# ehsankharazmi/hp-VPINNs

Measured on AMD Instinct MI355X. Metric: variational-loss iterations/sec, higher is better.
Workload: dtype f64; 1 GPU; Poisson-2D hp-VPINN, 16x16 elements, 20x20 GLL quad/elem, 10x10 test fcns/elem, MLP [2,20,20,20,1] tanh, var_form 1, 320 boundary pts, TF1 Adam (BASELINE config 4); points=102400, residuals=25600, params=921, backend=mfma, parallelism=element-sharded dp1, exchange=none, pass_structure=whole-iteration, kernel_variant=k_iter_fused<L=3,SPLIT=false,QT=true,GS=false>

## Files before the change

hp_vpinns_amd/csrc/kernels_fused.hip:

```cpp
#include <cstdio>
#include <cstdlib>
#include <cstring>
#include <type_traits>

#include "hpv_mfma_dev.h"
#include "hpv_fused_dev.h"

#define FZ_WAVES 4
#define FZ_BLOCK (FZ_WAVES * 64)
#define FZ_PRE_PER_THREAD 4
#define FZ_C 3
#define FZ_SHAPE_CONSTS                                                                                              \
    static constexpr int FZ_QX = QX_, FZ_QY = QY_, FZ_NTX = NTX_, FZ_NTY = NTY_, FZ_NQ = QX_ * QY_, FZ_NR = NTX_ * NTY_; \
    static constexpr int FZ_TPE = FZ_NQ / 16;                                                                        \
    static constexpr int FZ_MAXT = FZ_TPE / 4 + 1;       \
    static_assert(FZ_NQ % 16 == 0 && FZ_TPE % 4 <= 1, "element shape not covered by the whole-iteration kernel");
#define FZ_SHAPES(X) X(20, 20, 10, 10) X(16, 16, 8, 8) X(12, 12, 6, 6)

#ifdef HPV_FZ_TIMING
#define FZ_STAMP(I) fz_t[I] = clock64()
#define FZ_SEG(I) do { const long long t_ = clock64(); fz_seg[I] += t_ - fz_last; fz_last = t_; } while (0)
#else
#define FZ_STAMP(I)
#define FZ_SEG(I)
#endif

template <int L, int QX_, int QY_, int NTX_, int NTY_, bool MULTI = false, int C_ = FZ_C, int TRG_ = FZ_C, int NPART_ = 0>
struct FzLds {
    FZ_SHAPE_CONSTS
    static constexpr int LH = L > 1 ? L - 1 : 0;
    static constexpr int WT = 0;
    static constexpr int BH = WT + LH * MF_KS * 64;
    static constexpr int WR = BH + LH * MF_KS * 64;
    static constexpr int WN = WR + LH * MF_KS * 16;
    static constexpr int WRB = WN + LH * MF_KS * 64;
    static constexpr int W1O = WRB + LH * MF_KS * 16;
    static constexpr int CH = W1O + 4 * MF_KS * 64;
    static constexpr int PK = CH + 2 * FZ_NQ;
    static constexpr int XS = PK;
    static constexpr int XLD = FZ_NQ + 16;
    static constexpr int PKS = C_ > FZ_C ? 10 : 6;
    static constexpr int PP = PK + PKS * L * MF_KS * 64;
    static constexpr int PZ = PP + FZ_WAVES * NPART_ * 64;
    static constexpr int TR = PZ + (NPART_ > 0 ? 0 : FZ_WAVES * LH * MF_KS * 32);
    static constexpr int TR_WAVE = TRG_ * 2 * MF_TRB * MF_LD;
    static constexpr int TRSZ = FZ_WAVES * TR_WAVE;
    static constexpr int NTABS = 2 * FZ_NTX * FZ_QX + 2 * FZ_NTY * FZ_QY;
    static constexpr int AX = MULTI ? TR + TRSZ : TR;
    static constexpr int BY = AX + 2 * FZ_NTX * FZ_QX;
    static constexpr int T = MULTI ? TR : BY + 2 * FZ_NTY * FZ_QY;
    static constexpr int UP = T + 2 * FZ_QY * FZ_NTX;
    static constexpr int U = UP + 2 * FZ_NR;
    static constexpr int S = U + FZ_NR;
    static constexpr int RED = S + 2 * FZ_NTY * FZ_QX;
    static_assert(RED + 16 - TR <= FZ_WAVES * TR_WAVE, "projection scratch fits the transpose region");
    static_assert(3 * XLD <= 4 * L * MF_KS * 64, "the staged coordinates fit the parking slots the GS plan leaves free");
    static constexpr int EPI = NPART_ > 0 ? PK : TR;
    static constexpr int total(int P) { return NPART_ > 0 ? TR + TRSZ : TR + (TRSZ > FZ_WAVES * P ? TRSZ : FZ_WAVES * P) + (MULTI ? NTABS : 0); }
};
template <int L, int QX_, int QY_, int NT2>
struct FzPlan {
    static constexpr bool TIGHT = NT2 > 0 && L == 3 && QX_ * QY_ / 16 > 16;
    static constexpr int TRG = TIGHT ? 1 : (NT2 > 0 ? 2 : FZ_C);
    static constexpr int NPART = TIGHT ? 12 : 0;
};

typedef double v2d __attribute__((ext_vector_type(2)));
template <int L, bool SPLIT, bool QT, bool GS, int QX_, int QY_, int NTX_, int NTY_, bool MULTI = false, int NT2 = 0, bool GEN = false>
__global__ void __launch_bounds__(FZ_BLOCK, 1) k_iter_fused(MfmaArgs g) {
    static_assert(!(SPLIT && QT), "the quarter-tile scheme is for whole elements");
    static_assert(!(MULTI && (SPLIT || GS)), "the element loop is for whole elements on the register stash");
    static_assert(!((NT2 > 0 || GEN) && (GS || MULTI)), "the general forms run on the register stash, one workgroup (or a split) per element");
    static_assert(NT2 == 0 || GEN, "a second-tangent channel is always integrated through the general term weights");
    FZ_SHAPE_CONSTS
    static_assert(!(NT2 > 0 && QT && FZ_TPE % FZ_WAVES != 0), "four channels leave the packed quarter tile no slot for the data points: data-quarter plan only");
    constexpr int C = FZ_C + NT2;
    using PLAN = FzPlan<L, QX_, QY_, NT2>;
    constexpr int TRG = PLAN::TRG;
    constexpr int NPART = PLAN::NPART;
    static_assert(C % TRG == 0, "whole transpose passes");
    static_assert(NPART == 0 || !QT, "the tight plan: whole tiles");
    using M = FzLds<L, QX_, QY_, NTX_, NTY_, MULTI, C, TRG, NPART>;
    static_assert(!GEN || (M::AX == M::TR && 4 <= M::TR_WAVE), "the d-epsilon partials live in wave 0's part of the transpose region (it reads them back itself)");
    constexpr int LH = L > 1 ? L - 1 : 1;
    constexpr int NSV = L * MF_KS;
    extern __shared__ __attribute__((aligned(16))) double lds[];
    const int tid = threadIdx.x, lane = tid & 63;
    const int wv = __builtin_amdgcn_readfirstlane(tid >> 6);
    const int q = lane >> 4, pt = lane & 15;
    const int split = SPLIT ? g.proj_split : 1;
    const long el = SPLIT ? (long)(blockIdx.x % (unsigned)g.proj_n_elem) : (long)blockIdx.x;
    long e = SPLIT ? el + g.elem0 : el;
    const int part = SPLIT ? (int)(blockIdx.x / (unsigned)g.proj_n_elem) : 0;
    const double* __restrict__ th = g.theta;
    const ProjArgs& pa = g.pa;
#ifdef HPV_FZ_TIMING
    long long fz_t[8];
    const long long fz_start = clock64(), fz_wall = wall_clock64();
    long long fz_seg[2 + 2 * L], fz_last = clock64();
    int fz_n_own = 0;
#endif

    [[maybe_unused]] constexpr int TNX = FZ_NTX, TNY = FZ_NTY, TQX = FZ_QX, TQY = FZ_QY;
    const int rnx = pa.pd.ntx, rny = pa.pd.nty, rnr = rnx * rny;
    static_assert(FZ_NTX * FZ_QX == FZ_NTY * FZ_QY, "table staging walks both tables with one index");
    double bo = 0.0;
    auto stage_all = [&](auto th) {
        constexpr int N1 = 4 * MF_KS * 64, IT1 = (N1 + FZ_BLOCK - 1) / FZ_BLOCK;
        constexpr int ITW = (MF_KS * 64 + FZ_BLOCK - 1) / FZ_BLOCK;
        double vwt[L > 1 ? L - 1 : 1][ITW], vbh[L > 1 ? L - 1 : 1][ITW], vwn[L > 1 ? L - 1 : 1][ITW];
        double vwr[L > 1 ? L - 1 : 1], vwrb[L > 1 ? L - 1 : 1], v1[IT1];
#pragma unroll
        for (int i_ = 1; i_ < L; ++i_) {
            const int wo = g.woff[i_], bo_ = g.boff[i_];
#pragma unroll
            for (int it = 0; it < ITW; ++it) {
                const int f = it * FZ_BLOCK + tid, fc = f < MF_KS * 64 ? f : 0;
                const int ln = fc & 63, s_ = fc >> 6;
                vwt[i_ - 1][it] = th[wo + (4 * s_ + (ln >> 4)) * MF_H + (ln & 15)];
                vbh[i_ - 1][it] = th[bo_ + 4 * s_ + (ln >> 4)];
                vwn[i_ - 1][it] = th[wo + (ln & 15) * MF_H + 4 * s_ + (ln >> 4)];
            }
            const int fr = tid < MF_KS * 16 ? tid : 0;
            const int a_ = fr & 3, q_ = (fr >> 2) & 3, s_ = fr >> 4;
            vwr[i_ - 1] = th[wo + (4 * s_ + q_) * MF_H + 16 + a_];
            vwrb[i_ - 1] = th[wo + (16 + a_) * MF_H + 4 * s_ + q_];
        }
        const int w0o = g.woff[0], wLo = g.woff[L], b0o = g.boff[0];
#pragma unroll
        for (int it = 0; it < IT1; ++it) {
            const int f = it * FZ_BLOCK + tid, fc = f < N1 ? f : 0;
            const int ln = fc & 63, s_ = (fc >> 6) % MF_KS, c_ = fc / (64 * MF_KS);
            const int j = 4 * s_ + (ln >> 4);
            v1[it] = th[(c_ < 2 ? w0o + c_ * MF_H : (c_ == 2 ? wLo : b0o)) + j];
        }
        constexpr int NTAB = 2 * TNX * TQX, ITT = (NTAB + FZ_BLOCK - 1) / FZ_BLOCK;
        const int dx0 = pa.pd.t[0].dx, dx1 = pa.pd.t[1].dx, dy0 = pa.pd.t[0].dy, dy1 = pa.pd.t[1].dy;
        double vax[ITT], vby[ITT];
#pragma unroll
        for (int it = 0; it < ITT; ++it) {
            const int f = it * FZ_BLOCK + tid, fc = f < NTAB ? f : 0;
            const int tt_ = fc / (TNX * TQX), ti_ = fc % (TNX * TQX);
            const int rr_ = ti_ / TQX, ii_ = ti_ % TQX;
            const bool ton = !GEN || tt_ == 0 || pa.pd.nterms > 1;
            vax[it] = (rr_ < rnx && ton) ? pa.wtx[((long)(tt_ ? dx1 : dx0) * rnx + rr_) * TQX + ii_] : 0.0;
            vby[it] = (rr_ < rny && ton) ? pa.wty[((long)(tt_ ? dy1 : dy0) * rny + rr_) * TQY + ii_] : 0.0;
        }
#pragma unroll
        for (int i_ = 1; i_ < L; ++i_) {
#pragma unroll
            for (int it = 0; it < ITW; ++it) {
                const int f = it * FZ_BLOCK + tid;
                if (f < MF_KS * 64) {
                    lds[M::WT + (i_ - 1) * MF_KS * 64 + f] = vwt[i_ - 1][it];
                    lds[M::BH + (i_ - 1) * MF_KS * 64 + f] = vbh[i_ - 1][it];
                    lds[M::WN + (i_ - 1) * MF_KS * 64 + f] = vwn[i_ - 1][it];
                }
            }
            if (tid < MF_KS * 16) {
                lds[M::WR + (i_ - 1) * MF_KS * 16 + tid] = vwr[i_ - 1];
                lds[M::WRB + (i_ - 1) * MF_KS * 16 + tid] = vwrb[i_ - 1];
            }
        }
#pragma unroll
        for (int it = 0; it < IT1; ++it) {
            const int f = it * FZ_BLOCK + tid;
            if (f < N1) lds[M::W1O + f] = v1[it];
        }
#pragma unroll
        for (int it = 0; it < ITT; ++it) {
            const int f = it * FZ_BLOCK + tid;
            if (f < NTAB) { lds[M::AX + f] = vax[it]; lds[M::BY + f] = vby[it]; }
        }
        bo = th[g.boff[L]];
    };
    [[maybe_unused]] int pre_failed = -1;
    if constexpr (!GS && !MULTI) {
        if (g.pre_g) {
            double* TH = lds + M::PK;
            const AdamArgs& ad = g.pre_ad;
            const double flag = g.pre_g[g.pre_Ptot + 3];
            const int xe = *ad.xerr;
            const bool failed = !(flag == 0.0) || xe;
            pre_failed = failed ? 1 : 0;
            const double b1p = ad.state[0], b2p = ad.state[1];
            double t0[FZ_PRE_PER_THREAD], g0[FZ_PRE_PER_THREAD], m0[FZ_PRE_PER_THREAD], v0[FZ_PRE_PER_THREAD];
#pragma unroll
            for (int k = 0; k < FZ_PRE_PER_THREAD; ++k) {
                const int idx = tid + k * FZ_BLOCK;
                const bool in = idx < g.P;
                t0[k] = in ? ad.theta[idx] : 0.0; g0[k] = in ? g.pre_g[idx] : 0.0; m0[k] = in ? ad.m[idx] : 0.0; v0[k] = in ? ad.v[idx] : 1.0;
            }
#pragma unroll
            for (int k = 0; k < FZ_PRE_PER_THREAD; ++k) {
                const int idx = tid + k * FZ_BLOCK;
                double m1, v1, t1;
                hpv_adam_one(ad.lr, ad.b1, ad.b2, ad.eps, b1p, b2p, g0[k], m0[k], v0[k], t0[k], m1, v1, t1);
                if (idx < g.P) TH[idx] = failed ? t0[k] : t1;
            }
            if (blockIdx.x == 0 && tid == 0) {
                ad.xerr[1] = failed ? 1 : 0;
                if (failed && !xe) __hip_atomic_store(ad.xerr, 1, __ATOMIC_RELAXED, __HIP_MEMORY_SCOPE_AGENT);
            }
            __syncthreads();
            stage_all((const double*)TH);
        } else {
            stage_all(th);
        }
    } else {
        stage_all(th);
    }
    int xsticky = 0;
    unsigned xtag = 0;
    if constexpr (SPLIT) { xsticky = pre_failed >= 0 ? pre_failed : *g.xerr; xtag = *g.xiter + 1u; }
    double pc0 = pa.coef[e], pc1 = (!GEN || pa.pd.nterms > 1) ? pa.coef[pa.coef_stride + e] : 0.0;
    [[maybe_unused]] auto uni = [](double x) -> double {
        return __hiloint2double(__builtin_amdgcn_readfirstlane(__double2hiint(x)), __builtin_amdgcn_readfirstlane(__double2loint(x)));
    };
    [[maybe_unused]] const double geps = (GEN && pa.eps_ptr) ? uni(pa.eps_ptr[0]) : 0.0;
    [[maybe_unused]] const bool gtwo = GEN && pa.pd.nterms > 1;
    [[maybe_unused]] double WA0[C], WA1[C], WB1[C];
    if constexpr (GEN) {
#pragma unroll
        for (int c = 1; c < C; ++c) {
            const double t1 = uni(fma(geps, pa.pd.t[1].a1[c], pa.pd.t[1].a0[c]));
            WA0[c] = uni(fma(geps, pa.pd.t[0].a1[c], pa.pd.t[0].a0[c]));
            WA1[c] = uni(gtwo ? t1 : pa.pd.t[0].a1[c]);
            WB1[c] = uni(gtwo ? t1 : 0.0);
        }
    }
    [[maybe_unused]] auto wa0 = [&](int c) -> double { return WA0[c]; };
    [[maybe_unused]] auto wa1 = [&](int c) -> double { return WA1[c]; };
    [[maybe_unused]] auto wb1 = [&](int c) -> double { return WB1[c]; };
    [[maybe_unused]] const double gm0 = uni((GEN && pa.pd.t[0].eps_mult) ? geps : 1.0), gm1 = uni((gtwo && pa.pd.t[1].eps_mult) ? geps : 1.0);
    [[maybe_unused]] const double ge0 = (GEN && pa.pd.t[0].eps_mult) ? 1.0 : 0.0, ge1 = (gtwo && pa.pd.t[1].eps_mult) ? 1.0 : 0.0;
    const int ro_k = tid / FZ_NTX, ro_r = tid % FZ_NTX;
// ... 190 lines not shown
                    fz_layer<false>(lds + M::WT + (i - 1) * MF_KS * 64, lds + M::WR + (i - 1) * MF_KS * 16, nullptr, lofs, h[t][3], z[t][3]);
            }
            if constexpr (GS) {
#pragma unroll
                for (int t = 0; t < NT; ++t) {
                    v2d* zs = gs_ptr(tile_of(k0 + t)) + (i - 1) * MF_KS * 64;
#pragma unroll
                    for (int s = 0; s < MF_KS; ++s) zs[s * 64] = v2d{z[t][1][s], z[t][2][s]};
                }
            }
            [[maybe_unused]] double QZ[MF_KS];
            if constexpr (WQ)
                fz_layer_m(lds + M::WT + (i - 1) * MF_KS * 64, lds + M::WR + (i - 1) * MF_KS * 16, lds + M::BH + (i - 1) * MF_KS * 64, lofs,
                           q_tan ? 0.0 : 1.0, QH, QZ);
#pragma unroll
            for (int t = 0; t < NT; ++t)
#pragma unroll
                for (int s = 0; s < MF_KS; ++s) {
                    double a, a1, a2;
                    act_fwd<HPV_ACT_TANH>(z[t][0][s], a, a1, a2);
                    sv[t][i * MF_KS + s] = a;
                    h[t][0][s] = a; h[t][1][s] = a1 * z[t][1][s]; h[t][2][s] = a1 * z[t][2][s];
                    if constexpr (NT2 > 0)
                        h[t][3][s] = a2 * fma(g.t2w[0], z[t][1][s] * z[t][1][s], g.t2w[1] * (z[t][2][s] * z[t][2][s])) + a1 * z[t][3][s];
                }
            if constexpr (WQ) {
#pragma unroll
                for (int s = 0; s < MF_KS; ++s) {
                    double a, a1, a2;
                    act_fwd<HPV_ACT_TANH>(QZ[s], a, a1, a2);
                    const double a4 = dpp_move<0x114>(a), a8 = dpp_move<0x118>(a);
                    const double ab = qcs == 1 ? a4 : (qcs == 2 ? a8 : a);
                    QA[i * MF_KS + s] = ab;
                    QH[s] = q_tan ? (1.0 - ab * ab) * QZ[s] : ab;
                }
                if (q_tan) {
#pragma unroll
                    for (int s = 0; s < MF_KS; ++s) PKZ[((i - 1) * MF_KS + s) * 32 + q_cz] = QZ[s];
                }
            }
        }
#pragma unroll
        for (int t = 0; t < NT; ++t) {
            const int k = k0 + t;
            double o[C];
#pragma unroll
            for (int ch = 0; ch < C; ++ch) {
                double v = 0.0;
#pragma unroll
                for (int s = 0; s < MF_KS; ++s) v += h[t][ch][s] * lds[M::W1O + (2 * MF_KS + s) * 64 + lofs];
                v = xrow_sum16(v);
                v = xrow_sum32(v);
                o[ch] = v;
            }
            o[0] += bo;
            if (k < n_el) {
                if (q == 0) {
                    const int lp = (tbase + wv + k * FZ_WAVES) * 16 + pt;
                    double g0 = o[1], g1 = o[2];
                    if constexpr (GEN) {
                        g0 = 0.0; g1 = 0.0;
#pragma unroll
                        for (int c = 1; c < C; ++c) { g0 = fma(wa0(c), o[c], g0); g1 = fma(wa1(c), o[c], g1); }
                    }
                    if constexpr (SPLIT) {
                        if (!xstay) {
                            xg_publish(g.xg + (el * (2 * FZ_NQ) + lp) * 2, g0, xtag);
                            xg_publish(g.xg + (el * (2 * FZ_NQ) + FZ_NQ + lp) * 2, g1, xtag);
                        }
                    } else {
                        lds[M::CH + lp] = g0;
                        lds[M::CH + FZ_NQ + lp] = g1;
                    }
                }
            } else {
                double udv;
                if constexpr (GS) udv = lds[M::XS + 2 * M::XLD + pt]; else udv = valid[t] ? g.ud[pp[t] - g.data_off] : 0.0;
                const double dd = valid[t] ? udv - o[0] : 0.0;
                gdat = g.data_scale * dd;
                const double sq = row_sum16(dd * dd);
                if (lane == 0) g.data_part[pp[t] / 16 - g.data_off / 16] = sq;
            }
            stash(k, sv[t]);
        }
        if constexpr (WQ) {
            double v = 0.0;
#pragma unroll
            for (int s = 0; s < MF_KS; ++s) v += QH[s] * lds[M::W1O + (2 * MF_KS + s) * 64 + lofs];
            v = xrow_sum16(v);
            v = xrow_sum32(v);
            if constexpr (GEN && !DQ) {
                const double vo = dpp_move<0x104>(v), vm = dpp_move<0x114>(v);
                const double vx = qcs == 1 ? v : vm, vy = qcs == 1 ? vo : v;
                const double gq = qcs == 1 ? fma(wa0(1), vx, wa0(2) * vy) : fma(wa1(1), vx, wa1(2) * vy);
                if (q == 0 && q_tan) lds[M::CH + (qcs - 1) * FZ_NQ + q_lp] = gq;
            } else {
                if (!DQ && q == 0 && q_tan) lds[M::CH + (qcs - 1) * FZ_NQ + q_lp] = v;
            }
            const double dd = q_vdat ? qud - (v + bo) : 0.0;
            gdat_q = g.data_scale * dd;
            const double sq = row_sum16(q == 0 ? dd * dd : 0.0);
            if (lane == 0) lds[M::RED + 8 + wv] = sq;
            if (!q_tan) {
#pragma unroll
                for (int j = 0; j < NSV; ++j) PKQ[j * 32 + q_ci] = QA[j];
            }
        }
    };
    if constexpr (!GS) {
        load_x(0, xn[0], vn[0], pn[0]);
        load_x(1, xn[1], vn[1], pn[1]);
    }
    int k0 = 0;
    if constexpr (QT) {
        static_assert((FZ_TPE - (DQ ? 0 : 1)) / FZ_WAVES >= 2 && ((FZ_TPE - (DQ ? 0 : 1)) / FZ_WAVES) % 2 == 0, "trip plan of the QT instantiation: pairs of whole tiles");
#pragma unroll 1
        for (; k0 + 3 < n_own; k0 += 2) fwd_trip(k0, std::integral_constant<int, 2>{}, std::false_type{});
        fwd_trip(k0, std::integral_constant<int, 2>{}, std::true_type{});
    } else {
#pragma unroll 1
        for (; k0 + 1 < n_own; k0 += 2) fwd_trip(k0, std::integral_constant<int, 2>{}, std::false_type{});
        if (k0 < n_own) fwd_trip(k0, std::integral_constant<int, 1>{}, std::false_type{});
    }
    FZ_STAMP(2);
    if constexpr (SPLIT) {
        constexpr int NITG = (2 * FZ_NQ * 2 + FZ_BLOCK - 1) / FZ_BLOCK;
        bool ok = true;
        if (!xstay) ok = xg_gather<NITG, FZ_BLOCK>(g.xg + el * (2 * FZ_NQ) * 2, 2 * FZ_NQ * 2, xtag, (unsigned*)(lds + M::CH), tid);
        const int timed_out = __syncthreads_or(ok ? 0 : 1);
        if (timed_out || xstay) {
            if (timed_out && tid == 0) __hip_atomic_store(g.xerr, 1, __ATOMIC_RELAXED, __HIP_MEMORY_SCOPE_AGENT);
            return;
        }
    }
    if constexpr (GS && !SPLIT) pj_lds_barrier(); else __syncthreads();
    FZ_STAMP(3);
    [[maybe_unused]] v2d BA[GS ? NP : 1], BB[GS ? NP : 1];
    [[maybe_unused]] auto request = [&](int k, v2d (&B)[GS ? NP : 1]) {
        if constexpr (GS) {
            const v2d* zs = gs_ptr(tile_of(k));
            constexpr int NF = NZP + NSV / 2;
#pragma unroll
            for (int j = 0; j < NF; ++j) B[j] = zs[j * 64];
            if constexpr (NSV & 1) B[NF] = v2d{reinterpret_cast<const double*>(zs + NF * 64 - lane)[lane], 0.0};
        }
    };
    if constexpr (GS) { if (n_own > 0) request(0, BA); }
    if constexpr (QT) {
        if (tid == 0 && dtile < g.ntiles)
            g.data_part[dtile - g.data_off / 16] = (lds[M::RED + 8] + lds[M::RED + 9]) + (lds[M::RED + 10] + lds[M::RED + 11]);
    }

    {
        const double* G = lds + M::CH;
        int nax_e = FZ_NTX, nay_e = FZ_NTY;
        double nr_e = (double)rnr;
        if (pa.pd.nact) {
            nax_e = __builtin_amdgcn_readfirstlane(pa.pd.nact[e]);
            nay_e = __builtin_amdgcn_readfirstlane(pa.pd.nacty[e]);
            nr_e = (double)(nax_e * nay_e);
        }
        for (int o = tid; o < 2 * FZ_QY * FZ_NTX; o += FZ_BLOCK) {
            const int t = o / (FZ_QY * FZ_NTX), j = (o / FZ_NTX) % FZ_QY, r = o % FZ_NTX;
            const double* ax = lds + M::AX + (t * FZ_NTX + r) * FZ_QX;
            const double* gr = G + t * FZ_NQ + j * FZ_QX;
            double acc = 0.0;
#pragma unroll
            for (int i = 0; i < FZ_QX; ++i) acc = fma(ax[i], gr[i], acc);
            lds[M::T + o] = acc;
        }
        __syncthreads();
        if (tid < 2 * FZ_NR) {
            const int t = tid / FZ_NR, o = tid % FZ_NR, kk = o / FZ_NTX, r = o % FZ_NTX;
            const double* by = lds + M::BY + (t * FZ_NTY + kk) * FZ_QY;
            const double* tt = lds + M::T + t * FZ_QY * FZ_NTX + r;
            double acc = 0.0;
#pragma unroll
            for (int j = 0; j < FZ_QY; ++j) acc = fma(by[j], tt[j * FZ_NTX], acc);
            lds[M::UP + tid] = (t == 0 ? pc0 : pc1) * acc;
        }
        __syncthreads();
        double sq = 0.0;
        const double sc = 2.0 / nr_e;
        [[maybe_unused]] double deps = 0.0;
        if (tid < FZ_NR) {
            const bool act = ro_r < nax_e && ro_k < nay_e;
            double u;
            if constexpr (GEN) {
                const double u0 = lds[M::UP + tid], u1 = lds[M::UP + FZ_NR + tid];
                u = fma(gm0, u0, gm1 * u1) - pF;
                if (!act) u = 0.0;
                deps = sc * u * fma(ge0, u0, ge1 * u1);
            } else {
                u = (lds[M::UP + tid] + lds[M::UP + FZ_NR + tid]) - pF;
                if (!act) u = 0.0;
            }
            lds[M::U + tid] = u;
            if (ro_on) pa.R[ro_idx] = u;
            sq = u * u;
        }
        if (wv < 2) {
            sq = pj_wave_sum_dpp(sq);
            if (lane == 0) lds[M::RED + wv] = sq;
        }
        __syncthreads();
        if (tid == 0) pa.loss_e[e] = (lds[M::RED] + lds[M::RED + 1]) / nr_e;
        for (int o = tid; o < 2 * FZ_NTY * FZ_QX; o += FZ_BLOCK) {
            const int t = o / (FZ_NTY * FZ_QX), kk = (o / FZ_QX) % FZ_NTY, i = o % FZ_QX;
            const double* ax = lds + M::AX + t * FZ_NTX * FZ_QX + i;
            const double* ur = lds + M::U + kk * FZ_NTX;
            double acc = 0.0;
#pragma unroll
            for (int r = 0; r < FZ_NTX; ++r) acc = fma(ax[r * FZ_QX], ur[r], acc);
            if constexpr (GEN) lds[M::S + o] = acc * sc * (t == 0 ? pc0 * gm0 : pc1 * gm1);
            else lds[M::S + o] = acc * sc * (t == 0 ? pc0 : pc1);
        }
        __syncthreads();
        const int n_adj = (GEN && !gtwo) ? FZ_NQ : 2 * FZ_NQ;
        for (int o = tid; o < n_adj; o += FZ_BLOCK) {
            const int t = o / FZ_NQ, j = (o / FZ_QX) % FZ_QY, i = o % FZ_QX;
            const double* by = lds + M::BY + t * FZ_NTY * FZ_QY + j;
            const double* sr = lds + M::S + t * FZ_NTY * FZ_QX + i;
            double acc = 0.0;
#pragma unroll
            for (int kk = 0; kk < FZ_NTY; ++kk) acc = fma(by[kk * FZ_QY], sr[kk * FZ_QX], acc);
            if constexpr (GEN) { if (!gtwo) deps = fma(acc, lds[M::CH + FZ_NQ + o], deps); }
            lds[M::CH + o] = acc;
        }
        if constexpr (GEN) {
            if (pa.pd.has_eps) {
                deps = pj_wave_sum_dpp(deps);
                if (lane == 0) lds[M::AX + wv] = deps;
            }
        }
        __syncthreads();
        if constexpr (GEN) {
            if (pa.pd.has_eps && tid == 0) pa.deps_e[e] = (lds[M::AX] + lds[M::AX + 1]) + (lds[M::AX + 2] + lds[M::AX + 3]);
        }
    }

    FZ_STAMP(4);
    double* TAB = lds + M::TR + wv * M::TR_WAVE;
#pragma unroll
    for (int i = 0; i < LH; ++i) { dWacc[i] = v4d{0.0, 0.0, 0.0, 0.0}; dS10[i] = 0.0; dS01[i] = 0.0; accC[i] = 0.0; }
    dbo = 0.0;
#pragma unroll
    for (int s = 0; s < MF_KS; ++s) {
        dWo[s] = 0.0; dW1[0][s] = 0.0; dW1[1][s] = 0.0;
#pragma unroll
        for (int i = 0; i < L; ++i) db[i][s] = 0.0;
    }

#ifdef HPV_FZ_TIMING
    fz_last = clock64();
    fz_n_own = n_own;
    for (int i = 0; i < 2 + 2 * L; ++i) fz_seg[i] = 0;
#endif
    auto rev_tile = [&](int k, [[maybe_unused]] const v2d (&B)[GS ? NP : 1]) {
#ifdef HPV_FZ_TIMING
        fz_last = clock64();
#endif
        double x0, x1;
        if constexpr (GS) {
            const int lp = k < n_el ? (tbase + wv + k * FZ_WAVES) * 16 + pt : FZ_NQ + pt;
            x0 = lds[M::XS + lp]; x1 = lds[M::XS + M::XLD + lp];
        } else {
            const long tile = tile_of(k);
            const long p = tile * 16 + pt;
            const bool valid = p < g.N;
            x0 = valid ? g.X[p] : 0.0; x1 = valid ? g.X[g.N + p] : 0.0;
        }
        int lofs = lane;
        asm volatile("" : "+v"(lofs));
        double sv[NSV];
        if constexpr (GS) {
#pragma unroll
            for (int j = 0; j < NSV; ++j) sv[j] = B[NZP + j / 2][j & 1];
        } else if (k < n_lds) {
            const double* pk = k == 0 ? PKw : PKw2;
            if constexpr (NT2 > 0) pk = lds + M::PK + (k == 0 ? wv : (k == 1 ? 4 + wv : 8 + (wv & 1))) * (NSV * 64) + lane;
#pragma unroll
            for (int j = 0; j < NSV; ++j) sv[j] = pk[j * 64];
        } else {
            switch (k - n_lds) {
#define FZ_FETCH(K) case K: if constexpr (K < NREG) acc_get_all<AFULL + K * 2 * NSV, NSV>(sv); break;
                case 0:
                    if constexpr (NREG < 1) {
                    } else if constexpr (NPART > 0) {
                        const double* pp = lds + M::PP + wv * (NPART * 64) + lane;
#pragma unroll
                        for (int j = 0; j < NPART; ++j) sv[j] = pp[j * 64];
                        acc_get_from<ABASE, NSV, NPART>(sv);
                    } else {
                        acc_get_all<ABASE, NSV>(sv);
                    }
                    break;
                FZ_FETCH(1) FZ_FETCH(2) FZ_FETCH(3) FZ_FETCH(4)
#undef FZ_FETCH
                default:
#pragma unroll
                    for (int j = 0; j < NSV; ++j) sv[j] = 0.0;
            }
        }
        double gb[C];
        if (k < n_el) {
            const int lp = (tbase + wv + k * FZ_WAVES) * 16 + pt;
            gb[0] = 0.0; gb[1] = lds[M::CH + lp]; gb[2] = lds[M::CH + FZ_NQ + lp];
            if constexpr (GEN) {
                const double g0 = gb[1], g1 = gb[2];
#pragma unroll
                for (int c = 1; c < C; ++c) gb[c] = fma(wa0(c), g0, wb1(c) * g1);
            }
        } else {
            gb[0] = gdat; gb[1] = 0.0; gb[2] = 0.0;
            if constexpr (NT2 > 0) gb[3] = 0.0;
        }
        double zc[L][2][MF_KS];
        [[maybe_unused]] double zq[L][MF_KS];
        [[maybe_unused]] auto sq2 = [&](int i, int s) -> double { return fma(g.t2w[0], zc[i][0][s] * zc[i][0][s], g.t2w[1] * (zc[i][1][s] * zc[i][1][s])); };
#define ZC(I, CC, SS) zc[(I)][(CC)][(SS)]
#pragma unroll
        for (int s = 0; s < MF_KS; ++s) {
            zc[0][0][s] = lds[M::W1O + (0 * MF_KS + s) * 64 + lofs];
            zc[0][1][s] = lds[M::W1O + (1 * MF_KS + s) * 64 + lofs];
        }
#pragma unroll
        for (int i = 1; i < L; ++i) {
            if constexpr (GS) {
#pragma unroll
                for (int s = 0; s < MF_KS; ++s) { zc[i][0][s] = B[(i - 1) * MF_KS + s][0]; zc[i][1][s] = B[(i - 1) * MF_KS + s][1]; }
            } else {
                double hx[MF_KS], hy[MF_KS];
                [[maybe_unused]] double hq[MF_KS];
#pragma unroll
                for (int s = 0; s < MF_KS; ++s) {
                    const double a = sv[(i - 1) * MF_KS + s], a1 = 1.0 - a * a;
                    hx[s] = a1 * ZC(i - 1, 0, s); hy[s] = a1 * ZC(i - 1, 1, s);
                    if constexpr (NT2 > 0) hq[s] = (-2.0 * a * a1) * sq2(i - 1, s) + (i > 1 ? a1 * zq[i > 1 ? i - 1 : 0][s] : 0.0);
                }
                fz_layer<false>(lds + M::WT + (i - 1) * MF_KS * 64, lds + M::WR + (i - 1) * MF_KS * 16, nullptr, lofs, hx, zc[i][0]);
                fz_layer<false>(lds + M::WT + (i - 1) * MF_KS * 64, lds + M::WR + (i - 1) * MF_KS * 16, nullptr, lofs, hy, zc[i][1]);
                if constexpr (NT2 > 0) fz_layer<false>(lds + M::WT + (i - 1) * MF_KS * 64, lds + M::WR + (i - 1) * MF_KS * 16, nullptr, lofs, hq, zq[i]);
            }
        }

        FZ_SEG(0);
        double hbar[C][MF_KS], zbar[C][MF_KS];
        [[maybe_unused]] auto hv3 = [&](int i, int s) -> double {
            const double a = sv[i * MF_KS + s], a1 = 1.0 - a * a;
            return (-2.0 * a * a1) * sq2(i, s) + (i > 0 ? a1 * zq[i][s] : 0.0);
        };
#pragma unroll
        for (int s = 0; s < MF_KS; ++s) {
            const double a = sv[(L - 1) * MF_KS + s], a1 = 1.0 - a * a;
            const double wo = lds[M::W1O + (2 * MF_KS + s) * 64 + lofs];
            if (k >= n_el) dWo[s] = fma(a, gb[0], dWo[s]);
            dWo[s] = fma(a1 * zc[L - 1][0][s], gb[1], dWo[s]);
            dWo[s] = fma(a1 * zc[L - 1][1][s], gb[2], dWo[s]);
            hbar[0][s] = gb[0] * wo; hbar[1][s] = gb[1] * wo; hbar[2][s] = gb[2] * wo;
            if constexpr (NT2 > 0) { dWo[s] = fma(hv3(L - 1, s), gb[3], dWo[s]); hbar[3][s] = gb[3] * wo; }
        }
        if (q == 0) dbo += gb[0];
        FZ_SEG(1);

#pragma unroll
        for (int i = L - 1; i >= 0; --i) {
#pragma unroll
            for (int s = 0; s < MF_KS; ++s) {
                const double a = sv[i * MF_KS + s];
                const double a1 = 1.0 - a * a, a2 = -2.0 * a * a1;
                zbar[1][s] = hbar[1][s] * a1;
                zbar[2][s] = hbar[2][s] * a1;
                double zb = hbar[0][s] * a1 + a2 * (hbar[1][s] * ZC(i, 0, s) + hbar[2][s] * ZC(i, 1, s));
                if constexpr (NT2 > 0) {
                    const double hb = hbar[3][s], a3 = -2.0 * a1 * (1.0 - 3.0 * a * a);
                    zbar[3][s] = hb * a1;
                    zbar[1][s] = fma(2.0 * hb * a2 * g.t2w[0], ZC(i, 0, s), zbar[1][s]);
                    zbar[2][s] = fma(2.0 * hb * a2 * g.t2w[1], ZC(i, 1, s), zbar[2][s]);
                    zb = fma(hb, a3 * sq2(i, s) + (i > 0 ? a2 * zq[i][s] : 0.0), zb);
                }
                zbar[0][s] = zb;
                db[i][s] += zb;
            }
            if (i == 0) {
#pragma unroll
                for (int s = 0; s < MF_KS; ++s) {
                    dW1[0][s] += x0 * zbar[0][s] + zbar[1][s];
                    dW1[1][s] += x1 * zbar[0][s] + zbar[2][s];
                }
            } else {
// ... 1116 lines not shown
```

Measured before the change: 16790 it/s.

## Run per-element projection and adjoint contractions on f64 MFMA tiles

```diff
diff --git a/hp_vpinns_amd/csrc/kernels_fused.hip b/hp_vpinns_amd/csrc/kernels_fused.hip
--- a/hp_vpinns_amd/csrc/kernels_fused.hip
+++ b/hp_vpinns_amd/csrc/kernels_fused.hip
@@ -81,7 +81,6 @@
     static_assert(C % TRG == 0, "whole transpose passes");
     static_assert(NPART == 0 || !QT, "the tight plan: whole tiles");
     using M = FzLds<L, QX_, QY_, NTX_, NTY_, MULTI, C, TRG, NPART>;
-    static_assert(!GEN || (M::AX == M::TR && 4 <= M::TR_WAVE), "the d-epsilon partials live in wave 0's part of the transpose region (it reads them back itself)");
     constexpr int LH = L > 1 ? L - 1 : 1;
     constexpr int NSV = L * MF_KS;
     extern __shared__ __attribute__((aligned(16))) double lds[];
@@ -578,7 +577,6 @@
     }
 
     {
-        const double* G = lds + M::CH;
         int nax_e = FZ_NTX, nay_e = FZ_NTY;
         double nr_e = (double)rnr;
         if (pa.pd.nact) {
@@ -586,82 +584,206 @@
             nay_e = __builtin_amdgcn_readfirstlane(pa.pd.nacty[e]);
             nr_e = (double)(nax_e * nay_e);
         }
-        for (int o = tid; o < 2 * FZ_QY * FZ_NTX; o += FZ_BLOCK) {
-            const int t = o / (FZ_QY * FZ_NTX), j = (o / FZ_NTX) % FZ_QY, r = o % FZ_NTX;
-            const double* ax = lds + M::AX + (t * FZ_NTX + r) * FZ_QX;
-            const double* gr = G + t * FZ_NQ + j * FZ_QX;
-            double acc = 0.0;
-#pragma unroll
-            for (int i = 0; i < FZ_QX; ++i) acc = fma(ax[i], gr[i], acc);
-            lds[M::T + o] = acc;
-        }
-        __syncthreads();
-        if (tid < 2 * FZ_NR) {
-            const int t = tid / FZ_NR, o = tid % FZ_NR, kk = o / FZ_NTX, r = o % FZ_NTX;
-            const double* by = lds + M::BY + (t * FZ_NTY + kk) * FZ_QY;
-            const double* tt = lds + M::T + t * FZ_QY * FZ_NTX + r;
-            double acc = 0.0;
-#pragma unroll
-            for (int j = 0; j < FZ_QY; ++j) acc = fma(by[j], tt[j * FZ_NTX], acc);
-            lds[M::UP + tid] = (t == 0 ? pc0 : pc1) * acc;
-        }
-        __syncthreads();
-        double sq = 0.0;
-        const double sc = 2.0 / nr_e;
-        [[maybe_unused]] double deps = 0.0;
-        if (tid < FZ_NR) {
-            const bool act = ro_r < nax_e && ro_k < nay_e;
-            double u;
+        constexpr bool PJ_SCALAR = NT2 > 0 && FZ_NQ == 256;
+        if constexpr (PJ_SCALAR) {
+            static_assert(!GEN || (M::AX == M::TR && 4 <= M::TR_WAVE), "the d-epsilon partials live in wave 0's part of the transpose region (it reads them back itself)");
+            for (int o = tid; o < 2 * FZ_QY * FZ_NTX; o += FZ_BLOCK) {
+                const int t = o / (FZ_QY * FZ_NTX), j = (o / FZ_NTX) % FZ_QY, r = o % FZ_NTX;
+                const double* ax = lds + M::AX + (t * FZ_NTX + r) * FZ_QX;
+                const double* gr = lds + M::CH + t * FZ_NQ + j * FZ_QX;
+                double acc = 0.0;
+#pragma unroll
+                for (int i = 0; i < FZ_QX; ++i) acc = fma(ax[i], gr[i], acc);
+                lds[M::T + o] = acc;
+            }
+            __syncthreads();
+            if (tid < 2 * FZ_NR) {
+                const int t = tid / FZ_NR, o = tid % FZ_NR, kk = o / FZ_NTX, r = o % FZ_NTX;
+                const double* by = lds + M::BY + (t * FZ_NTY + kk) * FZ_QY;
+                const double* tt = lds + M::T + t * FZ_QY * FZ_NTX + r;
+                double acc = 0.0;
+#pragma unroll
+                for (int j = 0; j < FZ_QY; ++j) acc = fma(by[j], tt[j * FZ_NTX], acc);
+                lds[M::UP + tid] = (t == 0 ? pc0 : pc1) * acc;
+            }
+            __syncthreads();
+            double sq = 0.0;
+            const double sc = 2.0 / nr_e;
+            [[maybe_unused]] double deps = 0.0;
+            if (tid < FZ_NR) {
+                const bool act = ro_r < nax_e && ro_k < nay_e;
+                double u;
+                if constexpr (GEN) {
+                    const double u0 = lds[M::UP + tid], u1 = lds[M::UP + FZ_NR + tid];
+                    u = fma(gm0, u0, gm1 * u1) - pF;
+                    if (!act) u = 0.0;
+                    deps = sc * u * fma(ge0, u0, ge1 * u1);
+                } else {
+                    u = (lds[M::UP + tid] + lds[M::UP + FZ_NR + tid]) - pF;
+                    if (!act) u = 0.0;
+                }
+                lds[M::U + tid] = u;
+                if (ro_on) pa.R[ro_idx] = u;
+                sq = u * u;
+            }
+            if (wv < 2) {
+                sq = pj_wave_sum_dpp(sq);
+                if (lane == 0) lds[M::RED + wv] = sq;
+            }
+            __syncthreads();
+            if (tid == 0) pa.loss_e[e] = (lds[M::RED] + lds[M::RED + 1]) / nr_e;
+            for (int o = tid; o < 2 * FZ_NTY * FZ_QX; o += FZ_BLOCK) {
+                const int t = o / (FZ_NTY * FZ_QX), kk = (o / FZ_QX) % FZ_NTY, i = o % FZ_QX;
+                const double* ax = lds + M::AX + t * FZ_NTX * FZ_QX + i;
+                const double* ur = lds + M::U + kk * FZ_NTX;
+                double acc = 0.0;
+#pragma unroll
+                for (int r = 0; r < FZ_NTX; ++r) acc = fma(ax[r * FZ_QX], ur[r], acc);
+                if constexpr (GEN) lds[M::S + o] = acc * sc * (t == 0 ? pc0 * gm0 : pc1 * gm1);
+                else lds[M::S + o] = acc * sc * (t == 0 ? pc0 : pc1);
+            }
+            __syncthreads();
+            const int n_adj = (GEN && !gtwo) ? FZ_NQ : 2 * FZ_NQ;
+            for (int o = tid; o < n_adj; o += FZ_BLOCK) {
+                const int t = o / FZ_NQ, j = (o / FZ_QX) % FZ_QY, i = o % FZ_QX;
+                const double* by = lds + M::BY + t * FZ_NTY * FZ_QY + j;
+                const double* sr = lds + M::S + t * FZ_NTY * FZ_QX + i;
+                double acc = 0.0;
+#pragma unroll
+                for (int kk = 0; kk < FZ_NTY; ++kk) acc = fma(by[kk * FZ_QY], sr[kk * FZ_QX], acc);
+                if constexpr (GEN) { if (!gtwo) deps = fma(acc, lds[M::CH + FZ_NQ + o], deps); }
+                lds[M::CH + o] = acc;
+            }
             if constexpr (GEN) {
-                const double u0 = lds[M::UP + tid], u1 = lds[M::UP + FZ_NR + tid];
-                u = fma(gm0, u0, gm1 * u1) - pF;
-                if (!act) u = 0.0;
-                deps = sc * u * fma(ge0, u0, ge1 * u1);
-            } else {
-                u = (lds[M::UP + tid] + lds[M::UP + FZ_NR + tid]) - pF;
-                if (!act) u = 0.0;
-            }
-            lds[M::U + tid] = u;
-            if (ro_on) pa.R[ro_idx] = u;
-            sq = u * u;
-        }
-        if (wv < 2) {
-            sq = pj_wave_sum_dpp(sq);
-            if (lane == 0) lds[M::RED + wv] = sq;
-        }
-        __syncthreads();
-        if (tid == 0) pa.loss_e[e] = (lds[M::RED] + lds[M::RED + 1]) / nr_e;
-        for (int o = tid; o < 2 * FZ_NTY * FZ_QX; o += FZ_BLOCK) {
-            const int t = o / (FZ_NTY * FZ_QX), kk = (o / FZ_QX) % FZ_NTY, i = o % FZ_QX;
-            const double* ax = lds + M::AX + t * FZ_NTX * FZ_QX + i;
-            const double* ur = lds + M::U + kk * FZ_NTX;
-            double acc = 0.0;
-#pragma unroll
-            for (int r = 0; r < FZ_NTX; ++r) acc = fma(ax[r * FZ_QX], ur[r], acc);
-            if constexpr (GEN) lds[M::S + o] = acc * sc * (t == 0 ? pc0 * gm0 : pc1 * gm1);
-            else lds[M::S + o] = acc * sc * (t == 0 ? pc0 : pc1);
-        }
-        __syncthreads();
-        const int n_adj = (GEN && !gtwo) ? FZ_NQ : 2 * FZ_NQ;
-        for (int o = tid; o < n_adj; o += FZ_BLOCK) {
-            const int t = o / FZ_NQ, j = (o / FZ_QX) % FZ_QY, i = o % FZ_QX;
-            const double* by = lds + M::BY + t * FZ_NTY * FZ_QY + j;
-            const double* sr = lds + M::S + t * FZ_NTY * FZ_QX + i;
-            double acc = 0.0;
-#pragma unroll
-            for (int kk = 0; kk < FZ_NTY; ++kk) acc = fma(by[kk * FZ_QY], sr[kk * FZ_QX], acc);
-            if constexpr (GEN) { if (!gtwo) deps = fma(acc, lds[M::CH + FZ_NQ + o], deps); }
-            lds[M::CH + o] = acc;
-        }
-        if constexpr (GEN) {
-            if (pa.pd.has_eps) {
-                deps = pj_wave_sum_dpp(deps);
-                if (lane == 0) lds[M::AX + wv] = deps;
-            }
-        }
-        __syncthreads();
-        if constexpr (GEN) {
-            if (pa.pd.has_eps && tid == 0) pa.deps_e[e] = (lds[M::AX] + lds[M::AX + 1]) + (lds[M::AX + 2] + lds[M::AX + 3]);
+                if (pa.pd.has_eps) {
+                    deps = pj_wave_sum_dpp(deps);
+                    if (lane == 0) lds[M::AX + wv] = deps;
+                }
+            }
+            __syncthreads();
+            if constexpr (GEN) {
+                if (pa.pd.has_eps && tid == 0) pa.deps_e[e] = (lds[M::AX] + lds[M::AX + 1]) + (lds[M::AX + 2] + lds[M::AX + 3]);
+            }
+        } else {
+            constexpr int PJ_NJT = (FZ_QY + 15) / 16, PJ_NIT = (FZ_QX + 15) / 16;
+            constexpr int PJ_KX = FZ_QX / 4, PJ_KR = (FZ_NTX + 3) / 4, PJ_KK = (FZ_NTY + 3) / 4;
+            static_assert(FZ_QX % 4 == 0 && FZ_QY % 4 == 0 && FZ_NTX <= 16 && FZ_NTY <= 16, "projection tiles: whole k-steps over the points, one tile of test functions");
+            static_assert(2 * PJ_NJT * FZ_NR <= 2 * FZ_QY * FZ_NTX, "the partial sums of U fit the T array (T itself stays in registers)");
+            for (int u = wv; u < 2 * PJ_NJT; u += FZ_WAVES) {
+                const int t = u / PJ_NJT, jt = u % PJ_NJT;
+                const bool jon = jt * 16 + pt < FZ_QY, ron = pt < FZ_NTX, kon = pt < FZ_NTY;
+                const double* gr = lds + M::CH + t * FZ_NQ + (jon ? jt * 16 + pt : 0) * FZ_QX + q;
+                const double* ax = lds + M::AX + (t * FZ_NTX + (ron ? pt : 0)) * FZ_QX + q;
+                const double* by = lds + M::BY + (t * FZ_NTY + (kon ? pt : 0)) * FZ_QY + jt * 16 + q;
+                double ga[PJ_KX], xa[PJ_KX], ya[4];
+#pragma unroll
+                for (int s = 0; s < PJ_KX; ++s) { ga[s] = gr[4 * s]; xa[s] = ax[4 * s]; }
+#pragma unroll
+                for (int v = 0; v < 4; ++v) ya[v] = by[jt * 16 + 4 * v < FZ_QY ? 4 * v : 0];
+                v4d tt = v4d{0.0, 0.0, 0.0, 0.0};
+#pragma unroll
+                for (int s = 0; s < PJ_KX; ++s)
+                    tt = __builtin_amdgcn_mfma_f64_16x16x4f64(jon ? ga[s] : 0.0, ron ? xa[s] : 0.0, tt, 0, 0, 0);
+                v4d up = v4d{0.0, 0.0, 0.0, 0.0};
+#pragma unroll
+                for (int v = 0; v < 4; ++v)
+                    if (jt * 16 + 4 * v < FZ_QY)
+                        up = __builtin_amdgcn_mfma_f64_16x16x4f64(kon ? ya[v] : 0.0, tt[v], up, 0, 0, 0);
+#pragma unroll
+                for (int v = 0; v < 4; ++v)
+                    if (q + 4 * v < FZ_NTY && ron) lds[M::T + u * FZ_NR + (q + 4 * v) * FZ_NTX + pt] = up[v];
+            }
+            pj_lds_barrier();
+            double sq = 0.0;
+            const double sc = 2.0 / nr_e;
+            [[maybe_unused]] double deps = 0.0;
+            auto up_t = [&](int t) -> double {
+                double a = lds[M::T + t * PJ_NJT * FZ_NR + tid];
+#pragma unroll
+                for (int jt = 1; jt < PJ_NJT; ++jt) a += lds[M::T + (t * PJ_NJT + jt) * FZ_NR + tid];
+                return a;
+            };
+            if (tid < FZ_NR) {
+                const bool act = ro_r < nax_e && ro_k < nay_e;
+                double u;
+                if constexpr (GEN) {
+                    const double u0 = pc0 * up_t(0), u1 = pc1 * up_t(1);
+                    u = fma(gm0, u0, gm1 * u1) - pF;
+                    if (!act) u = 0.0;
+                    deps = sc * u * fma(ge0, u0, ge1 * u1);
+                } else {
+                    u = (pc0 * up_t(0) + pc1 * up_t(1)) - pF;
+                    if (!act) u = 0.0;
+                }
+                lds[M::U + tid] = u;
+                if (ro_on) pa.R[ro_idx] = u;
+                sq = u * u;
+            }
+            if (wv < 2) {
+                sq = pj_wave_sum_dpp(sq);
+                if (lane == 0) lds[M::RED + wv] = sq;
+            }
+            pj_lds_barrier();
+            if (tid == 0) pa.loss_e[e] = (lds[M::RED] + lds[M::RED + 1]) / nr_e;
+            const int n_adj = (GEN && !gtwo) ? PJ_NIT : 2 * PJ_NIT;
+            for (int u = wv; u < n_adj; u += FZ_WAVES) {
+                const int t = u / PJ_NIT, it = u % PJ_NIT;
+                const int i = it * 16 + pt;
+                const bool ion = i < FZ_QX, kon = pt < FZ_NTY;
+                const double* ur = lds + M::U + (kon ? pt : 0) * FZ_NTX;
+                const double* ax = lds + M::AX + t * FZ_NTX * FZ_QX + (ion ? i : 0);
+                double ua[PJ_KR], xa[PJ_KR];
+#pragma unroll
+                for (int s = 0; s < PJ_KR; ++s) {
+                    const int rc = 4 * s + q < FZ_NTX ? 4 * s + q : 0;
+                    ua[s] = ur[rc]; xa[s] = ax[rc * FZ_QX];
+                }
+                v4d ss = v4d{0.0, 0.0, 0.0, 0.0};
+#pragma unroll
+                for (int s = 0; s < PJ_KR; ++s) {
+                    const bool ron = 4 * s + q < FZ_NTX;
+                    ss = __builtin_amdgcn_mfma_f64_16x16x4f64((kon && ron) ? ua[s] : 0.0, (ron && ion) ? xa[s] : 0.0, ss, 0, 0, 0);
+                }
+#pragma unroll
+                for (int v = 0; v < 4; ++v) {
+                    if constexpr (GEN) ss[v] = ss[v] * sc * (t == 0 ? pc0 * gm0 : pc1 * gm1);
+                    else ss[v] = ss[v] * sc * (t == 0 ? pc0 : pc1);
+                }
+#pragma unroll
+                for (int jt = 0; jt < PJ_NJT; ++jt) {
+                    const int j = jt * 16 + pt;
+                    const bool jon = j < FZ_QY;
+                    const double* by = lds + M::BY + t * FZ_NTY * FZ_QY + (jon ? j : 0);
+                    v4d gg = v4d{0.0, 0.0, 0.0, 0.0};
+#pragma unroll
+                    for (int v = 0; v < PJ_KK; ++v) {
+                        const bool k4 = 4 * v + q < FZ_NTY;
+                        const double b = by[(k4 ? 4 * v + q : 0) * FZ_QY];
+                        gg = __builtin_amdgcn_mfma_f64_16x16x4f64((k4 && jon) ? b : 0.0, ss[v], gg, 0, 0, 0);
+                    }
+#pragma unroll
+                    for (int v = 0; v < 4; ++v) {
+                        const int jo = jt * 16 + q + 4 * v;
+                        if (jo < FZ_QY && ion) {
+                            const int o = jo * FZ_QX + i;
+                            if constexpr (GEN) { if (!gtwo) deps = fma(gg[v], lds[M::CH + FZ_NQ + o], deps); }
+                            lds[M::CH + t * FZ_NQ + o] = gg[v];
+                        }
+                    }
+                }
+            }
+            if constexpr (GEN) {
+                if (pa.pd.has_eps) {
+                    deps = pj_wave_sum_dpp(deps);
+                    if (lane == 0) lds[M::UP + wv] = deps;
+                }
+            }
+            __syncthreads();
+            if constexpr (GEN) {
+                constexpr int PJ_DW = (M::UP - M::TR) / M::TR_WAVE;
+                static_assert(PJ_DW < FZ_WAVES && M::UP + FZ_WAVES - M::TR <= (PJ_DW + 1) * M::TR_WAVE, "the d-epsilon partials live in one wave's part of the transpose region");
+                if (pa.pd.has_eps && tid == PJ_DW * 64) pa.deps_e[e] = (lds[M::UP] + lds[M::UP + 1]) + (lds[M::UP + 2] + lds[M::UP + 3]);
+            }
         }
     }
 
```

Result: faster. 16970 it/s, median of 6 (+1.1%).
